# juanmc2005/diart

Hardware: NVIDIA H100
Metric: audio-seconds/sec (real-time factor) at 5s/0.5s step, batch 256 (higher is better)
Workload: dtype f32

## Files before the change

### diart_b200/_lib.py

```python
from __future__ import annotations

import ctypes as C
import os
from typing import Dict, Optional

import numpy as np
import torch

_HERE = os.path.dirname(os.path.abspath(__file__))
LIB_PATH = os.path.join(_HERE, "libdiartb200.so")

_lib: Optional[C.CDLL] = None


class DgTensor(C.Structure):
    _fields_ = [("name", C.c_char_p), ("data", C.c_void_p), ("numel", C.c_int64)]


_P = C.c_void_p
SIGNATURES = {
    "dg_last_error": (C.c_char_p, []),
    "dg_version": (C.c_int, []),
    "dg_launch_count": (C.c_int64, []),
    "dg_profile_enable": (C.c_int, [C.c_int]),
    "dg_profile_report": (C.c_int, [C.c_char_p, C.c_int]),
    "dg_selftest_gemm_tc": (C.c_int, [C.c_int, C.c_int, C.c_int, C.c_int, C.c_int, C.c_int, C.POINTER(C.c_float),
                                      C.POINTER(C.c_float)]),
    "dg_selftest_gemm_tc_grid": (C.c_int, [C.c_int, C.c_int, C.c_int, C.c_int, C.c_int, C.c_int, C.POINTER(C.c_int)]),
    "dg_selftest_gemm_tc_bounds": (C.c_int, [C.c_int, C.c_int, C.c_int, C.c_int, C.POINTER(C.c_int), C.POINTER(C.c_int),
                                             C.POINTER(C.c_int)]),
    "dg_selftest_wgmma_row_shift": (C.c_int, [C.c_int, C.POINTER(C.c_uint)]),
    "dg_selftest_gemm_tc_halo": (C.c_int, [C.c_int, C.c_int, C.c_int, C.c_int, C.c_int, C.c_int, C.POINTER(C.c_int),
                                           C.POINTER(C.c_int)]),
    "dg_selftest_split_f16_host": (C.c_int, [_P, C.c_longlong, _P, _P]),
    "dg_seg_create": (C.c_int, [C.POINTER(DgTensor), C.c_int, C.c_int, C.POINTER(_P)]),
    "dg_seg_dims": (C.c_int, [_P, C.c_int, C.POINTER(C.c_int), C.POINTER(C.c_int)]),
    "dg_seg_set_powerset": (C.c_int, [_P, C.c_int, C.c_int]),
    "dg_seg_forward": (C.c_int, [_P, _P, C.c_int, C.c_int, _P, _P]),
    "dg_seg_destroy": (C.c_int, [_P]),
    "dg_emb_create": (C.c_int, [C.POINTER(DgTensor), C.c_int, C.c_int, C.c_int, C.POINTER(_P)]),
    "dg_emb_dims": (C.c_int, [_P, C.c_int, C.POINTER(C.c_int), C.POINTER(C.c_int)]),
    "dg_emb_forward": (C.c_int, [_P, _P, _P, C.c_int, C.c_int, C.c_int, C.c_int, C.c_int, C.c_float, _P, _P]),
    "dg_emb_forward_rows": (C.c_int, [_P, _P, _P, C.c_int, C.c_int, C.c_int, _P, _P]),
    "dg_emb_destroy": (C.c_int, [_P]),
    "dg_emb_debug_trunk": (C.c_int, [_P, _P, C.c_int, C.c_int, C.c_int, _P, C.c_int64, _P]),
    "dg_seg_debug_stage": (C.c_int, [_P, _P, C.c_int, C.c_int, C.c_int, C.c_int, _P, C.c_int64, _P]),
    "dg_emb_debug_stage": (C.c_int, [_P, _P, _P, C.c_int, C.c_int, C.c_int, C.c_int, C.c_int, C.c_int, _P, C.c_int64, _P]),
    "dg_selftest_sinc_filters_host": (C.c_int, [_P, _P, _P]),
    "dg_selftest_fbank_tables_host": (C.c_int, [_P, _P]),
    "dg_osp": (C.c_int, [_P, C.c_int, C.c_int, C.c_int, C.c_float, C.c_float, C.c_int, _P, _P]),
    "dg_normalize_embeddings": (C.c_int, [_P, C.c_int, C.c_int, C.c_float, _P, _P]),
    "dg_cluster_create": (C.c_int, [C.c_int, C.c_int, C.c_double, C.c_double, C.c_double, C.c_int, C.POINTER(_P)]),
    "dg_cluster_set_metric": (C.c_int, [_P, C.c_int]),
    "dg_cluster_step": (C.c_int, [_P, _P, _P, C.c_int, C.c_int, C.c_int, _P, _P, _P]),
    "dg_cluster_reset": (C.c_int, [_P]),
# ... 149 lines not shown
```

### diart_b200/csrc/api.cu

```cuda
#include <math.h>
#include <stdlib.h>
#include <string.h>

#include <map>
#include <sstream>
#include <vector>

#include "host.cuh"

namespace dg {

static thread_local std::string g_err;
std::atomic<long long> g_launches{0};
thread_local int g_sm_limit = 0;
void set_error(const std::string& msg) { g_err = msg; }

struct ProfRec {
  std::string name;
  cudaEvent_t a, b;
};
static bool g_prof = false;
static std::vector<ProfRec> g_recs;
static const bool g_trace = getenv("DG_TRACE_LAUNCHES") && getenv("DG_TRACE_LAUNCHES")[0] == '1';
ProfScope::ProfScope(const char* name_, cudaStream_t st_) : on(g_prof), st(st_), a(nullptr), b(nullptr), name(name_) {
// ... 342 lines not shown
  ref.tap_boxes = 1;
  if (folded) {
    ref.Cin = Kf;
    ref.KW = 1;
    if ((rc = set_weights(ref, dWf))) return rc;
  }
  std::vector<unsigned char> first, cur;
  *equal = 1;
  for (int run = 0; run < 3; run++) {
    DG_CUDA(cudaMemset(dF.p, 0, f32_bytes + 4));
    DG_CUDA(cudaMemset(dOh.p, 0, plane_bytes + 4));
    DG_CUDA(cudaMemset(dOl.p, 0, plane_bytes + 4));
    DG_CUDA(cudaMemset(dPart.p, 0, part_bytes + 4));
    {
      SmLimit cap(run == 1 ? 3 : 0);
      if ((rc = launch_gemm_tc(run == 2 ? ref : t, nullptr))) return rc;
    }
    DG_CUDA(cudaDeviceSynchronize());
    cur.resize(f32_bytes + 2 * plane_bytes + part_bytes);
    DG_CUDA(cudaMemcpy(cur.data(), dF.p, f32_bytes, cudaMemcpyDeviceToHost));
    DG_CUDA(cudaMemcpy(cur.data() + f32_bytes, dOh.p, plane_bytes, cudaMemcpyDeviceToHost));
    DG_CUDA(cudaMemcpy(cur.data() + f32_bytes + plane_bytes, dOl.p, plane_bytes, cudaMemcpyDeviceToHost));
    DG_CUDA(cudaMemcpy(cur.data() + f32_bytes + 2 * plane_bytes, dPart.p, part_bytes, cudaMemcpyDeviceToHost));
    if (run == 0)
      first.swap(cur);
    else if (cur != first)
      *equal = 0;
  }
  return DG_OK;
}

extern "C" int dg_selftest_gemm_tc_bounds(int M, int Cin, int N, int epi, int* outside_unchanged, int* equal, int* refused) {
  const bool planes = epi == 1;
  if (M < 1 || Cin < 64 || Cin % 64 || N < 1 || N % (planes ? 32 : 4) || epi < 0 || epi > 2 || !outside_unchanged || !equal ||
      !refused) {
    set_error("dg_selftest_gemm_tc_bounds: bad arguments");
    return DG_EINVAL;
  }
  const int npad = N <= 64 && epi == 0 ? 64 : (N + 127) / 128 * 128, esize = planes ? 2 : 4;
  const int ldc = N + 40;
  const long long rows = (long long)M + 130;
  uint32_t seed = 4242u;
  auto rnd = [&]() {
    seed = seed * 1664525u + 1013904223u;
    return ((seed >> 8) & 0xFFFF) / 65536.f - 0.5f;
  };
// ... 64 lines not shown
```

### diart_b200/csrc/dg_common.cuh

```cuda
#pragma once
#include <cuda_runtime.h>
#include <stdint.h>
#include <stdio.h>

#include <atomic>
#include <string>
#include <vector>

namespace dg {

void set_error(const std::string& msg);
extern std::atomic<long long> g_launches;
extern thread_local int g_sm_limit;
inline int usable_sms() {
  int dev = 0, sms = 132;
  cudaGetDevice(&dev);
  cudaDeviceGetAttribute(&sms, cudaDevAttrMultiProcessorCount, dev);
  return (g_sm_limit > 0 && g_sm_limit < sms) ? g_sm_limit : sms;
}

#define DG_CUDA(expr)                                                                   \
  do {                                                                                  \
    cudaError_t _e = (expr);                                                            \
    if (_e != cudaSuccess) {                                                            \
// ... 100 lines not shown
  float* out_f32;
  void* out_hi;
  void* out_lo;
  int ldc;
  int epi;
  const char* tag;
  const int* tap_off;
  int Wp, Hp, Wop, Hop, stride2, relu;
  const void* res_hi;
  const void* res_lo;
  const float* pool_w;
  float* pool_part;
  int pool_item_rows, pool_K;
  int pool3_T, pool3_tile_rows;
  int tap_boxes;
};
inline int gemm_tc_pool3_tile_rows(int item_rows) {
  for (int t = 126; t >= 96; t -= 3)
    if (item_rows % t == 0) return t;
  return 0;
}
int launch_gemm_tc(const TcGemm& g, cudaStream_t st);
bool gemm_tc_halo(const TcGemm& g);
int selftest_wgmma_row_shift(int base_offset_mode, unsigned* ok_shifts);
int launch_split_ex(const float* x, long long rows_out, int C, int ld_in, int ld_out, int pool, int item_rows,
                    const float* sc, const float* sh, void* hi, void* lo, cudaStream_t st, const int* skip_flag = nullptr);
void split_weights_host(const float* w, int N, int Npad, int K, uint16_t* hi, uint16_t* lo, float scale = 1.f);
float weight_plane_scale(const float* w, size_t n);
uint16_t host_f32_to_h16(float f);
float host_h16_to_f32(uint16_t h);
int sinc_tc_rows_per_item(const Geom& g);
size_t sinc_tc_plane_elems(int B, const Geom& g);
void sinc_tc_pack_filters(const float* filt, uint16_t* planes );
void sinc_tc_affine_consts(const float* filt, float beta, float* cf);
int launch_sinc_prep(const float* wav, const float* mean, const float* rstd, int B, const Geom& g, void* planes_hi,
                     void* planes_lo, cudaStream_t st, const int* skip_flag = nullptr);
int launch_sinc0_tc(float gamma, const float* cf_dev, const void* w_planes, int B, const Geom& g, const void* planes_hi,
                    const void* planes_lo, float* p0, cudaStream_t st, const int* skip_flag = nullptr);
struct SincStreamGeom {
  int Ls;
  int P;
  int rows;
  size_t plane;
};
SincStreamGeom sinc_stream_geom(int B, const Geom& g, int hop);
int launch_overlap_check(const float* wav, int B, int S, int hop, int* flag, cudaStream_t st);
// ... 148 lines not shown
```

### diart_b200/csrc/gemm_tc.cu

```cuda
#include <cuda.h>
#include <cuda_bf16.h>
#include <math.h>
#include <stdlib.h>
#include <string.h>

#include <algorithm>
#include <map>
#include <mutex>
#include <string>
#include <utility>
#include <vector>

#include "dg_common.cuh"
#include "tc_ptx.cuh"

namespace dg {

constexpr int TC_BM = 128, TC_BK = 32, TC_THREADS = 384;
constexpr int TC_SMEM_MAX = 227 * 1024;

struct TcArgs {
  long long M;
  int N;
  int m_tiles, n_tiles;
  int KW, dil, cin_blocks;
  const float* bias;
  const float* bn_scale;
  const float* bn_shift;
  float* out_f32;
  __nv_bfloat16* out_hi;
  __nv_bfloat16* out_lo;
  int ldc;
  float acc_scale;
  int tap_off[9];
  int Wp, Hp, Wop, Hop, stride2, relu;
  const __nv_bfloat16* res_hi;
  const __nv_bfloat16* res_lo;
  const float* pool_w;
  float* pool_part;
  int pool_item_rows, pool_K;
  int tile_rows, pool3_T;
  unsigned* tile_ctr;
  int halo_rows;
  int cin;
  int wblocks;
  int halo_bytes;
  int op_bytes;
};

enum TcEpi { TC_BIAS_F32 = 0, TC_LEAKY_BN_SPLIT = 1, TC_LEAKY_BN_F32 = 2, TC_CONV2D = 3, TC_POOL = 4, TC_MAXPOOL3 = 5 };

__host__ __device__ constexpr bool tc_pooling(int epi) { return epi == TC_POOL || epi == TC_MAXPOOL3; }
__host__ __device__ constexpr bool tc_box_store(int epi) { return epi == TC_BIAS_F32 || epi == TC_LEAKY_BN_SPLIT || epi == TC_LEAKY_BN_F32; }

template <int BN>
struct TcSmem {
  static constexpr int A_BYTES = TC_BM * TC_BK * 2;
  static constexpr int W_BYTES = BN * TC_BK * 2;
  static constexpr int STAGE_BYTES = 2 * A_BYTES + 2 * W_BYTES;
  static constexpr int W_STAGE_BYTES = 2 * W_BYTES;
  static constexpr int NSTAGE = BN == 128 ? 4 : 6;
  static constexpr int NSTAGE_HALO = BN == 128 ? 5 : 6;
  __host__ static int halo_bytes(int cin, int rows) { return (2 * ((cin + 31) / 32) * rows * 64 + 1023) / 1024 * 1024; }
  __host__ static int halo_op_bytes(int cin, int rows) { return 2 * halo_bytes(cin, rows) + NSTAGE_HALO * W_STAGE_BYTES; }
  static constexpr int BAR_BYTES = 256;
  static constexpr int PARAM_FLOATS = 3 * BN;
  static constexpr int CHUNK_W = 64;
  static constexpr int CHUNK_FLOATS = CHUNK_W / 32 * TC_BM * 33;
  __host__ __device__ static constexpr int extra_floats(int epi) { return epi == TC_POOL ? 128 * 4 + 4 * 2 * 8 * 32 : (epi == TC_MAXPOOL3 ? 4 * 2 * 2 * 32 : 0); }
  __host__ __device__ static constexpr int consumer_floats(int epi) { return PARAM_FLOATS + (tc_pooling(epi) ? CHUNK_FLOATS + extra_floats(epi) : 0); }
  static constexpr int ACC_LD = BN + 4;
  static constexpr int BOX_BYTES = TC_BM * 128;
  __host__ __device__ static constexpr int stage_tile_bytes(int epi) {
    return tc_pooling(epi) ? 0 : (epi == TC_CONV2D ? TC_BM * ACC_LD * 4 : TC_BM * BN * 4);
  }
  __host__ __device__ static constexpr int total(int epi, int op_bytes = NSTAGE * STAGE_BYTES) {
    return op_bytes + stage_tile_bytes(epi) + BAR_BYTES + 2 * consumer_floats(epi) * 4 + 1024;
  }
};
static_assert(TcSmem<128>::total(TC_POOL) <= TC_SMEM_MAX && TcSmem<64>::total(TC_MAXPOOL3) <= TC_SMEM_MAX &&
              TcSmem<128>::total(TC_CONV2D) <= TC_SMEM_MAX && TcSmem<64>::total(TC_CONV2D) <= TC_SMEM_MAX &&
              TcSmem<32>::total(TC_CONV2D) <= TC_SMEM_MAX && TcSmem<128>::total(TC_BIAS_F32) <= TC_SMEM_MAX,
              "gemm_tc: shared memory");

template <int BN, int EPI>
__device__ __forceinline__ void tc_stage_params(const TcArgs& a, float* params, int bar, int n0, int et) {
  named_sync(bar, 128);
  for (int i = et; i < BN; i += 128) {
    const int n = n0 + i;
    const bool ok = n < a.N;
    params[i] = (ok && a.bias) ? a.bias[n] : 0.f;
    constexpr bool has_bn = EPI != TC_BIAS_F32;
    params[BN + i] = (ok && has_bn) ? a.bn_scale[n] * (EPI == TC_CONV2D ? a.acc_scale : 1.f) : 1.f;
    params[2 * BN + i] = (ok && has_bn) ? a.bn_shift[n] : 0.f;
  }
  named_sync(bar, 128);
}

template <int BN, int EPI>
__device__ __forceinline__ void tc_box_epilogue(const TcArgs& a, const float* params, float (&acc)[2][BN / 2],
                                                uint32_t tile, int quad, int lane) {
  using S = TcSmem<BN>;
  const int r0 = 16 * quad + (lane >> 2), sw = lane >> 2, cq = lane & 3;
#pragma unroll
  for (int j = 0; j < BN / 8; j++) {
    const int col = 8 * j + 2 * cq;
    const float2 bias = *reinterpret_cast<const float2*>(params + col);
    float2 bsc = make_float2(1.f, 1.f), bsh = make_float2(0.f, 0.f);
    if (EPI != TC_BIAS_F32) {
      bsc = *reinterpret_cast<const float2*>(params + BN + col);
      bsh = *reinterpret_cast<const float2*>(params + 2 * BN + col);
    }
#pragma unroll
    for (int h = 0; h < 2; h++) {
#pragma unroll
      for (int e2 = 0; e2 < 2; e2++) {
        const int row = 64 * h + r0 + 8 * e2;
        float x0 = fmaf(acc[h][4 * j + 2 * e2], a.acc_scale, bias.x);
        float x1 = fmaf(acc[h][4 * j + 2 * e2 + 1], a.acc_scale, bias.y);
        if (EPI != TC_BIAS_F32) {
          x0 = fmaf(leaky(x0), bsc.x, bsh.x);
          x1 = fmaf(leaky(x1), bsc.y, bsh.y);
        }
        if (EPI == TC_LEAKY_BN_SPLIT) {
          uint16_t h0, l0, h1, l1;
          split_h16(x0, h0, l0);
          split_h16(x1, h1, l1);
          const int off = (j / 8) * S::BOX_BYTES + row * 128 + (((j & 7) ^ sw) << 4) + 4 * cq;
          st_shared_u32(tile + off, pack_u16x2(h0, h1));
          st_shared_u32(tile + (BN / 64) * S::BOX_BYTES + off, pack_u16x2(l0, l1));
        } else {
          const int q = 2 * (j & 3) + (cq >> 1);
          const int off = (j / 4) * S::BOX_BYTES + row * 128 + ((q ^ sw) << 4) + 8 * (cq & 1);
          st_shared_v2(tile + off, x0, x1);
        }
      }
    }
  }
}

__device__ __forceinline__ void acc_ld32(const float* p, uint32_t (&r)[32]) {
#pragma unroll
  for (int i = 0; i < 8; i++) {
    const float4 v = reinterpret_cast<const float4*>(p)[i];
    r[4 * i] = __float_as_uint(v.x);
    r[4 * i + 1] = __float_as_uint(v.y);
    r[4 * i + 2] = __float_as_uint(v.z);
    r[4 * i + 3] = __float_as_uint(v.w);
  }
}

template <int BN>
__device__ __forceinline__ void tc_conv2d_epilogue_tile(const TcArgs& a, const float* params, const float* acc_row,
                                                        long long mt, int n0, int quad, int lane) {
    const long long m = mt * TC_BM + quad * 32 + lane;
    long long mo = m;
// ... 204 lines not shown
                }
              }
            }
#pragma unroll
            for (int sg = 0; sg < 2; sg++) {
              stg[((rg * 2 + sg) * 2 + 0) * 32 + col] = s1[sg];
              stg[((rg * 2 + sg) * 2 + 1) * 32 + col] = s2[sg];
            }
          }
          named_sync(bar, 128);
          {
            const int col = et & 31, q = et >> 5, sg = q >> 1, j = q & 1, n = n0 + c + col;
            const float tot = ((stg[((0 * 2 + sg) * 2 + j) * 32 + col] + stg[((1 * 2 + sg) * 2 + j) * 32 + col]) +
                               stg[((2 * 2 + sg) * 2 + j) * 32 + col]) + stg[((3 * 2 + sg) * 2 + j) * 32 + col];
            if (n < a.N) a.pool_part[(((size_t)mt * 2 + sg) * 2 + j) * a.N + n] = tot;
          }
          named_sync(bar, 128);
          continue;
        }
      }
    }
}

template <int BN, int EPI, bool HALO>
__global__ void __launch_bounds__(TC_THREADS, 1)
gemm_tc_kernel(const __grid_constant__ CUtensorMap tmA_hi, const __grid_constant__ CUtensorMap tmA_lo,
               const __grid_constant__ CUtensorMap tmW_hi, const __grid_constant__ CUtensorMap tmW_lo,
               const __grid_constant__ CUtensorMap tmC0, const __grid_constant__ CUtensorMap tmC1, TcArgs a) {
  using S = TcSmem<BN>;
  constexpr bool POOLING = tc_pooling(EPI);
  constexpr int NSTAGE = HALO ? S::NSTAGE_HALO : S::NSTAGE;
  extern __shared__ unsigned char smem_raw[];
  unsigned char* smem = reinterpret_cast<unsigned char*>((reinterpret_cast<uintptr_t>(smem_raw) + 1023) & ~uintptr_t(1023));
  unsigned char* ring = HALO ? smem + 2 * a.halo_bytes : smem;
  constexpr int RING_STAGE = HALO ? S::W_STAGE_BYTES : S::STAGE_BYTES;
  unsigned char* tile_s = smem + a.op_bytes;
  uint64_t* bars = reinterpret_cast<uint64_t*>(tile_s + S::stage_tile_bytes(EPI));
  uint64_t* full = bars;
  uint64_t* empty = bars + NSTAGE;
  uint64_t* tile_full = bars + 2 * NSTAGE;
  uint64_t* tile_empty = tile_full + 2;
  uint64_t* halo_full = tile_empty + 2;
  uint64_t* halo_empty = halo_full + 2;
  volatile int* tile_idx = reinterpret_cast<volatile int*>(halo_empty + 2);
  float* cons = reinterpret_cast<float*>(reinterpret_cast<unsigned char*>(bars) + S::BAR_BYTES);

  const int warp = __shfl_sync(0xffffffffu, (int)(threadIdx.x >> 5), 0), lane = threadIdx.x & 31;
  const int wg = warp >> 2;
  const int num_tiles = a.m_tiles * a.n_tiles;
  const int kblocks = HALO ? a.wblocks : a.KW * a.cin_blocks;
  const int halo_box = a.halo_rows * 64, halo_cb = (a.cin + 31) / 32;

  if (threadIdx.x == 0) {
    for (int s = 0; s < NSTAGE; s++) {
      mbar_init(&full[s], 1);
      mbar_init(&empty[s], 1);
    }
    for (int c = 0; c < 2; c++) {
      mbar_init(&tile_full[c], 1);
      mbar_init(&tile_empty[c], 128);
      mbar_init(&halo_full[c], 1);
      mbar_init(&halo_empty[c], 1);
    }
    asm volatile("fence.mbarrier_init.release.cluster;" ::: "memory");
  }
  __syncthreads();

  if (wg == 0) {
    setmaxnreg_dec<HALO ? 48 : 40>();
    if (threadIdx.x == 0) {
      int stage = 0, phase = 0, next = 0;
      bool halo_next = false;
      for (int i = 0, tile = blockIdx.x;; i++) {
        const int c = i & 1;
        mbar_wait(&tile_empty[c], ((i >> 1) & 1) ^ 1);
        if (tile >= num_tiles) {
          tile_idx[c] = -1;
          mbar_arrive(&tile_full[c]);
          mbar_wait(&tile_empty[c ^ 1], (((i + 1) >> 1) & 1) ^ 1);
          tile_idx[c ^ 1] = -2;
          mbar_arrive(&tile_full[c ^ 1]);
          break;
        }
        tile_idx[c] = tile;
        mbar_arrive(&tile_full[c]);
        const int mt = tile / a.n_tiles, nt = tile - mt * a.n_tiles;
        const int m0 = mt * (EPI == TC_MAXPOOL3 ? a.tile_rows : TC_BM), n0 = nt * BN;
        if constexpr (HALO) {
          auto load_halo = [&](int cc, int r0) {
            unsigned char* hs = smem + cc * a.halo_bytes;
            mbar_expect_tx(&halo_full[cc], 2 * halo_cb * halo_box);
            for (int cb = 0; cb < halo_cb; cb++) {
              tma_load_2d(hs + cb * halo_box, &tmA_hi, cb * TC_BK, r0, &halo_full[cc]);
              tma_load_2d(hs + (halo_cb + cb) * halo_box, &tmA_lo, cb * TC_BK, r0, &halo_full[cc]);
            }
// ... 9 lines not shown
          for (int kb = 0; kb < kblocks; kb++) {
            const long long t0 = clock64();
            for (;;) {
              if (!halo_next && next < num_tiles && mbar_test_wait(&halo_empty[c ^ 1], next_par)) {
                load_halo(c ^ 1, next_m0);
                halo_next = true;
              }
              if (mbar_test_wait(&empty[stage], phase ^ 1)) break;
              if (clock64() - t0 > 4000000000LL) __trap();
            }
            unsigned char* st = ring + stage * RING_STAGE;
            mbar_expect_tx(&full[stage], S::W_STAGE_BYTES);
            tma_load_2d(st, &tmW_hi, kb * TC_BK, n0, &full[stage]);
            tma_load_2d(st + S::W_BYTES, &tmW_lo, kb * TC_BK, n0, &full[stage]);
            if (++stage == NSTAGE) {
              stage = 0;
              phase ^= 1;
            }
          }
        }
        for (int j = 0; j < (HALO ? 0 : a.KW); j++) {
          for (int cb = 0; cb < a.cin_blocks; cb++) {
            mbar_wait(&empty[stage], phase ^ 1);
            unsigned char* st = smem + stage * S::STAGE_BYTES;
            mbar_expect_tx(&full[stage], S::STAGE_BYTES);
            const int kcol = (j * a.cin_blocks + cb) * TC_BK;
            tma_load_2d(st, &tmA_hi, cb * TC_BK, m0 + a.tap_off[j], &full[stage]);
            tma_load_2d(st + S::A_BYTES, &tmA_lo, cb * TC_BK, m0 + a.tap_off[j], &full[stage]);
            tma_load_2d(st + 2 * S::A_BYTES, &tmW_hi, kcol, n0, &full[stage]);
            tma_load_2d(st + 2 * S::A_BYTES + S::W_BYTES, &tmW_lo, kcol, n0, &full[stage]);
            if (++stage == NSTAGE) {
              stage = 0;
              phase ^= 1;
            }
          }
        }
        if (!HALO) next = POOLING ? (int)gridDim.x + (int)atomicAdd(&a.tile_ctr[0], 1u) : tile + (int)gridDim.x;
        tile = next;
      }
      if (POOLING) {
        __threadfence();
        if (atomicAdd(&a.tile_ctr[1], 1u) == gridDim.x - 1) {
          atomicExch(&a.tile_ctr[0], 0u);
          atomicExch(&a.tile_ctr[1], 0u);
        }
      }
    }
    return;
  }
  setmaxnreg_inc<HALO ? 224 : 232>();
  const int c = wg - 1, quad = warp & 3, et = threadIdx.x - 128 * wg;
  float* params = cons + c * S::consumer_floats(EPI);
  float* chunk = params + S::PARAM_FLOATS;
  float* pool_stage = chunk + S::CHUNK_FLOATS;
  const int bar = 1 + c, turn = 3 + c, turn_other = 3 + (c ^ 1), acc_free = 5 + c, acc_free_other = 5 + (c ^ 1);
  if (c == 1) {
    named_arrive(3, 256);
    if (!POOLING) named_arrive(5, 256);
  }
  for (int n = 0;; n++) {
    mbar_wait(&tile_full[c], n & 1);
    const int tile = tile_idx[c];
    mbar_arrive(&tile_empty[c]);
    if (tc_box_store(EPI) && tile >= 0 && (a.n_tiles > 1 || n == 0))
      tc_stage_params<BN, EPI>(a, params, bar, (tile - tile / a.n_tiles * a.n_tiles) * BN, et);
    named_sync(turn, 256);
    if (tile < 0) {
      if (tile == -1) {
        named_arrive(turn_other, 256);
        if (!POOLING) named_sync(acc_free, 256);
      }
      break;
    }
    const int pos = (2 * n + c) * kblocks;
    int stage = pos % NSTAGE, phase = (pos / NSTAGE) & 1;
    float acc[2][BN / 2];
#pragma unroll
    for (int i = 0; i < BN / 2; i++) acc[0][i] = acc[1][i] = 0.f;
    uint32_t htap = 0;
    int hch = 0;
    if constexpr (HALO) mbar_wait(&halo_full[c], n & 1);
    const uint32_t hs = smem_u32(smem + c * a.halo_bytes);
    for (int kb = 0; kb < kblocks; kb++) {
      mbar_wait(&full[stage], phase);
      const uint32_t sa = smem_u32(ring + stage * RING_STAGE);
      const uint32_t sw = HALO ? sa : sa + 2 * S::A_BYTES;
      const uint64_t w_hi = wg_desc_sw64(sw), w_lo = wg_desc_sw64(sw + S::W_BYTES);
      constexpr uint64_t HALF = (uint64_t)((64 * TC_BK * 2) >> 4);
      wg_fence_acc(acc[0]);
      wg_fence_acc(acc[1]);
      wg_fence();
#pragma unroll
      for (int ks = 0; ks < TC_BK / 16; ks++) {
        const uint64_t adv = (uint64_t)((ks * 32) >> 4);
        uint64_t a_hi, a_lo;
        if constexpr (HALO) {
          const uint32_t aa = hs + (uint32_t)(hch >> 5) * halo_box + (uint32_t)(hch & 31) * 2 + htap;
          a_hi = wg_desc_sw64(aa);
          a_lo = wg_desc_sw64(aa + halo_cb * halo_box);
          hch += 16;
          const bool next_tap = hch == a.cin;
          hch = next_tap ? 0 : hch;
          htap += next_tap ? a.dil * 64 : 0;
        } else {
          a_hi = wg_desc_sw64(sa) + adv;
          a_lo = wg_desc_sw64(sa + S::A_BYTES) + adv;
        }
#pragma unroll
        for (int h = 0; h < 2; h++) {
          wgmma_ss<BN>(acc[h], a_lo + h * HALF, w_hi + adv, (kb | ks) != 0);
          wgmma_ss<BN>(acc[h], a_hi + h * HALF, w_lo + adv, 1);
          wgmma_ss<BN>(acc[h], a_hi + h * HALF, w_hi + adv, 1);
        }
      }
      wg_commit();
      wg_wait<1>();
      wg_fence_acc(acc[0]);
      wg_fence_acc(acc[1]);
      if (kb > 0 && et == 0) mbar_arrive(&empty[stage == 0 ? NSTAGE - 1 : stage - 1]);
      if (++stage == NSTAGE) {
        stage = 0;
        phase ^= 1;
      }
    }
    named_arrive(turn_other, 256);
    wg_wait<0>();
    wg_fence_acc(acc[0]);
    wg_fence_acc(acc[1]);
    if (et == 0) mbar_arrive(&empty[stage == 0 ? NSTAGE - 1 : stage - 1]);
    if (HALO && et == 0) mbar_arrive(&halo_empty[c]);
    const int mt = tile / a.n_tiles, nt = tile - mt * a.n_tiles;
    const bool stage_params = a.n_tiles > 1 || n == 0;
    if constexpr (POOLING) {
      tc_pool_epilogue_tile<BN, EPI>(a, params, chunk, pool_stage, acc, bar, mt, nt * BN, quad, lane, et, stage_params);
    } else if constexpr (EPI == TC_CONV2D) {
      float* acc_s = reinterpret_cast<float*>(tile_s);
      named_sync(acc_free, 256);
#pragma unroll
      for (int h = 0; h < 2; h++) {
        const int r0 = 64 * h + 16 * quad + (lane >> 2);
#pragma unroll
        for (int j = 0; j < BN / 8; j++) {
          const int col = 8 * j + 2 * (lane & 3);
          *reinterpret_cast<float2*>(acc_s + r0 * S::ACC_LD + col) = make_float2(acc[h][4 * j], acc[h][4 * j + 1]);
          *reinterpret_cast<float2*>(acc_s + (r0 + 8) * S::ACC_LD + col) = make_float2(acc[h][4 * j + 2], acc[h][4 * j + 3]);
        }
      }
      named_sync(bar, 128);
      if (stage_params) tc_stage_params<BN, EPI>(a, params, bar, nt * BN, et);
      tc_conv2d_epilogue_tile<BN>(a, params, acc_s + et * S::ACC_LD, mt, nt * BN, quad, lane);
      named_arrive(acc_free_other, 256);
    } else {
      named_sync(acc_free, 256);
      tc_box_epilogue<BN, EPI>(a, params, acc, smem_u32(tile_s), quad, lane);
      fence_proxy_async_smem();
      named_sync(bar, 128);
      if (et == 0) {
        const int m0 = mt * TC_BM, n0 = nt * BN;
        if (EPI == TC_LEAKY_BN_SPLIT) {
#pragma unroll
          for (int b = 0; b < BN / 64; b++) {
            if (n0 + 64 * b >= a.N) break;
            tma_store_2d(&tmC0, tile_s + b * S::BOX_BYTES, n0 + 64 * b, m0);
            tma_store_2d(&tmC1, tile_s + (BN / 64 + b) * S::BOX_BYTES, n0 + 64 * b, m0);
          }
        } else {
#pragma unroll
          for (int b = 0; b < BN / 32; b++) {
            if (n0 + 32 * b >= a.N) break;
            tma_store_2d(&tmC0, tile_s + b * S::BOX_BYTES, n0 + 32 * b, m0);
          }
        }
        bulk_commit();
// ... 57 lines not shown
  }
  void* base = nullptr;
  if (cudaGetSymbolAddress(&base, g_tc_tile_ctr) != cudaSuccess) {
    set_error("gemm_tc: cannot address the tile counters");
    return nullptr;
  }
  return static_cast<unsigned*>(base) + 2 * slot;
}

static int tc_bn(const TcGemm& g) { return g.epi == TC_MAXPOOL3 || (g.Npad == 64 && g.epi == TC_BIAS_F32) ? 64 : 128; }
static int tc_halo_rows(const TcGemm& g) {
  return (TC_BM + (g.KW - ((g.KW * g.Cin) % 32 ? 0 : 1)) * g.dil + 7) / 8 * 8;
}
template <int BN>
static int tc_halo_smem(const TcGemm& g) { return TcSmem<BN>::total(g.epi, TcSmem<BN>::halo_op_bytes(g.Cin, tc_halo_rows(g))); }

bool gemm_tc_halo(const TcGemm& g) {
  if (g.tap_boxes || g.epi == TC_CONV2D || g.tap_off || g.KW < 2 || g.dil < 1 || g.Cin % 16 || g.Cin > 128 ||
      tc_halo_rows(g) > 256)
    return false;
  return (tc_bn(g) == 64 ? tc_halo_smem<64>(g) : tc_halo_smem<128>(g)) <= TC_SMEM_MAX;
}

static int tc_setup(const TcGemm& g, int bn, int epi, bool halo, CUtensorMap* maps, TcArgs& a) {
  const int Ktot = g.KW * g.Cin, bk = TC_BK, a_rows = halo ? tc_halo_rows(g) : TC_BM;
  if (make_map(&maps[0], g.A_hi, g.Mtot, g.Cin, g.lda, bk, a_rows) || make_map(&maps[1], g.A_lo, g.Mtot, g.Cin, g.lda, bk, a_rows) ||
      make_map(&maps[2], g.W_hi, g.Npad, Ktot, Ktot, bk, bn) || make_map(&maps[3], g.W_lo, g.Npad, Ktot, Ktot, bk, bn))
    return -2;
  memset(&maps[4], 0, 2 * sizeof(CUtensorMap));
  if (epi == TC_LEAKY_BN_SPLIT) {
    if (make_map(&maps[4], g.out_hi, g.M, g.N, g.ldc, 64, TC_BM) || make_map(&maps[5], g.out_lo, g.M, g.N, g.ldc, 64, TC_BM))
      return -2;
  } else if (tc_box_store(epi)) {
    if (make_map(&maps[4], g.out_f32, g.M, g.N, g.ldc, 32, TC_BM, true)) return -2;
  }
  a = TcArgs{};
  a.M = g.M; a.N = g.N; a.n_tiles = (g.N + bn - 1) / bn;
  a.tile_rows = epi == TC_MAXPOOL3 ? g.pool3_tile_rows : TC_BM;
  a.pool3_T = g.pool3_T;
  a.m_tiles = (int)((g.M + a.tile_rows - 1) / a.tile_rows);
  a.KW = g.KW; a.dil = g.dil; a.cin_blocks = g.Cin / bk;
  a.bias = g.bias; a.bn_scale = g.bn_scale; a.bn_shift = g.bn_shift;
  a.out_f32 = g.out_f32; a.out_hi = reinterpret_cast<__nv_bfloat16*>(g.out_hi);
  a.out_lo = reinterpret_cast<__nv_bfloat16*>(g.out_lo); a.ldc = g.ldc;
  a.acc_scale = g.w_scale > 0.f ? 1.f / g.w_scale : 1.f;
  for (int j = 0; j < 9; j++) a.tap_off[j] = j < g.KW ? (g.tap_off ? g.tap_off[j] : j * g.dil) : 0;
  a.Wp = g.Wp; a.Hp = g.Hp; a.Wop = g.Wop; a.Hop = g.Hop; a.stride2 = g.stride2; a.relu = g.relu;
  a.res_hi = reinterpret_cast<const __nv_bfloat16*>(g.res_hi);
  a.res_lo = reinterpret_cast<const __nv_bfloat16*>(g.res_lo);
  a.pool_w = g.pool_w; a.pool_part = g.pool_part; a.pool_item_rows = g.pool_item_rows; a.pool_K = g.pool_K;
  a.cin = g.Cin;
  if (halo) {
    a.halo_rows = a_rows;
    a.wblocks = (Ktot + bk - 1) / bk;
    a.halo_bytes = bn == 64 ? TcSmem<64>::halo_bytes(g.Cin, a_rows) : TcSmem<128>::halo_bytes(g.Cin, a_rows);
    a.op_bytes = bn == 64 ? TcSmem<64>::halo_op_bytes(g.Cin, a_rows) : TcSmem<128>::halo_op_bytes(g.Cin, a_rows);
  } else {
    a.op_bytes = bn == 128 ? TcSmem<128>::NSTAGE * TcSmem<128>::STAGE_BYTES
                           : (bn == 64 ? TcSmem<64>::NSTAGE * TcSmem<64>::STAGE_BYTES : TcSmem<32>::NSTAGE * TcSmem<32>::STAGE_BYTES);
  }
  return 0;
}

static int tc_grid(const TcArgs& a) {
  const int sms = usable_sms();
  const int tiles = a.m_tiles * a.n_tiles;
  return tiles < sms ? tiles : sms;
}

template <int BN, int EPI, bool HALO>
static int launch_tc(const TcGemm& g, cudaStream_t st) {
  using S = TcSmem<BN>;
  CUtensorMap m[6];
  TcArgs a;
  if (tc_setup(g, BN, EPI, HALO, m, a)) return -2;
  if (tc_pooling(EPI) && !(a.tile_ctr = tile_counter(st))) return -2;
  auto kern = gemm_tc_kernel<BN, EPI, HALO>;
  static bool attr_done[64] = {};
  if (first_use_on_device(attr_done))
    DG_CUDA(cudaFuncSetAttribute(kern, cudaFuncAttributeMaxDynamicSharedMemorySize, HALO ? TC_SMEM_MAX : S::total(EPI)));
  kern<<<tc_grid(a), TC_THREADS, S::total(EPI, a.op_bytes), st>>>(m[0], m[1], m[2], m[3], m[4], m[5], a);
  DG_LAUNCHED();
  return 0;
}

template <int BN, int EPI>
static int launch_tc(const TcGemm& g, cudaStream_t st) {
  return gemm_tc_halo(g) ? launch_tc<BN, EPI, true>(g, st) : launch_tc<BN, EPI, false>(g, st);
}

int launch_gemm_tc(const TcGemm& g, cudaStream_t st) {
  ProfScope _ps(g.tag ? g.tag : "gemm_tc", st);
  if (g.Cin % (gemm_tc_halo(g) ? 16 : 64) || g.lda % 8 || g.ldc % (g.epi == TC_LEAKY_BN_SPLIT ? 8 : 4) ||
      (g.Npad % 128 && g.Npad != 64 && g.Npad != 32) || g.KW < 1 || g.KW > 9) {
    set_error("gemm_tc: Cin must be a multiple of 64 (a Conv1d of 2..9 taps over at most 128 channels whose tile halo fits "
              "in shared memory, e.g. Cin 80: a multiple of 16), A pitch a multiple of 8, output pitch a multiple of 4 "
              "(8 for 16-bit planes), padded N 32, 64 or a multiple of 128, at most 9 taps");
    return -1;
  }
  if (g.epi == TC_LEAKY_BN_SPLIT && g.N % 32) {
    set_error("gemm_tc (planes): N must be a multiple of 32");
    return -1;
  }
  if (tc_box_store(g.epi)) {
    const bool planes = g.epi == TC_LEAKY_BN_SPLIT;
    const uintptr_t base = planes ? ((uintptr_t)g.out_hi | (uintptr_t)g.out_lo) : (uintptr_t)g.out_f32;
    if (!base || (planes && (!g.out_hi || !g.out_lo)) || base % 16 || g.ldc < g.N || g.M >= (1LL << 31)) {
      set_error("gemm_tc: the output needs a 16-byte aligned base, a pitch of at least N and fewer than 2^31 rows");
      return -1;
    }
  }
  if (g.epi == TC_CONV2D) {
    if (g.ldc % 32 || g.N % 32 || g.Wp < 3 || g.Hp < 3 || (!g.out_hi && !g.out_f32) || g.M >= (1LL << 31)) {
      set_error("gemm_tc (conv2d): channel counts must be multiples of 32");
      return -1;
    }
    if (g.Npad == 32) return launch_tc<32, TC_CONV2D, false>(g, st);
    if (g.Npad == 64) return launch_tc<64, TC_CONV2D, false>(g, st);
    return launch_tc<128, TC_CONV2D, false>(g, st);
  }
// ... 220 lines not shown
```

### include/diart_b200.h

```cpp
#ifndef DIART_B200_H
#define DIART_B200_H

#include <stddef.h>
#include <stdint.h>

#ifdef __cplusplus
extern "C" {
#endif

#define DG_OK 0
#define DG_EINVAL (-1)
#define DG_ECUDA (-2)
#define DG_EWEIGHT (-3)
#define DG_ENCCL (-4)

typedef struct dg_tensor {
  const char* name;
  const float* data;
  int64_t numel;
} dg_tensor;

typedef struct dg_seg dg_seg;
typedef struct dg_emb dg_emb;
typedef struct dg_cluster dg_cluster;
// ... 156 lines not shown
int dg_selftest_multi_frames_host(int slots, int max_wps, int out_chunk, int out_step, int n_rates, const int32_t* rates,
                                  int n_ops, const int32_t* ops, int32_t* result, int64_t* records, int cap, int* n_records);
int dg_selftest_multi_staging_host(int slots, int C, int n_ops, const int32_t* ops, const float* samples_host, int32_t* result,
                                   float* rings_host);
int dg_multi_create_vad(dg_seg* seg, int chunk_samples, int step_samples, int max_streams, int max_windows_per_stream,
                        double tau, int num_windows, const double* hamming_host, dg_multi** out);

typedef struct dg_resample dg_resample;
int dg_resample_create(int orig_rate, int new_rate, const float* taps_host, int width, int device, dg_resample** out);
int64_t dg_resample_out_len(const dg_resample* h, int64_t num_samples);
int dg_resample_forward(dg_resample* h, const float* in_dev, int B, int64_t L, float* out_dev, void* stream);
int dg_resample_destroy(dg_resample* h);
int dg_stream_create_resampled(int chunk_samples, int step_samples, dg_resample* rs, int max_windows, int device,
                               dg_stream** out);
int dg_stream_crop_host(dg_stream* h, int n, const int64_t* ranges_host, float* out_host);

int64_t dg_launch_count(void);
int dg_profile_enable(int enable);
int dg_selftest_gemm_tc(int M, int Cin, int KW, int dil, int N, int epi, float* max_abs_diff, float* out_rms);
int dg_selftest_gemm_tc_grid(int M, int Cin, int KW, int dil, int N, int epi, int* equal);
int dg_selftest_gemm_tc_bounds(int M, int Cin, int N, int epi, int* outside_unchanged, int* equal, int* refused);
int dg_selftest_wgmma_row_shift(int base_offset_mode, unsigned* ok_shifts);
int dg_selftest_gemm_tc_halo(int M, int Cin, int KW, int dil, int N, int epi, int* equal, int* halo);
int dg_selftest_split_f16_host(const float* x, long long n, unsigned short* hi, unsigned short* lo);
int dg_selftest_sinc_filters_host(const float* low_hz, const float* band_hz, float* filters);
int dg_selftest_fbank_tables_host(float* frame_operator, float* mel_banks);
int dg_profile_report(char* buf, int cap);

int dg_cluster_record_len(const dg_cluster* h);
int dg_cluster_export_delta(dg_cluster* h, double* record_dev, void* stream);
int dg_cluster_merge(dg_cluster* h, const double* records_dev , int world, int rank,
                     int32_t* maps_dev , int n_maps, void* stream);
int dg_pipeline_identity_export(dg_pipeline* h, double* record_dev, void* stream);
int dg_pipeline_identity_merge(dg_pipeline* h, const double* records_dev, int world, int rank, void* stream);

#ifdef __cplusplus
}
#endif
#endif
```

Before: 23120.

## Add weight-resident mode to tensor-core GEMM keeping the full weight slice in shared memory

Adds a weight-resident variant of the persistent wgmma GEMM for 1-tap, BN=128, box-store epilogues. Each CTA loads its entire N-column weight slice into shared memory once and then streams only A tiles through a smaller ring. The grid is pinned so each CTA keeps a fixed n-tile. The epilogue is split into narrower column passes to shrink the staging tile. This cuts repeated weight TMA traffic per k-block but leaves fewer pipeline stages, can reduce grid size, and serializes epilogue stores.

```diff
diff --git a/diart_b200/_lib.py b/diart_b200/_lib.py
--- a/diart_b200/_lib.py
+++ b/diart_b200/_lib.py
@@ -31,6 +31,8 @@
                                              C.POINTER(C.c_int)]),
     "dg_selftest_wgmma_row_shift": (C.c_int, [C.c_int, C.POINTER(C.c_uint)]),
     "dg_selftest_gemm_tc_halo": (C.c_int, [C.c_int, C.c_int, C.c_int, C.c_int, C.c_int, C.c_int, C.POINTER(C.c_int),
+                                           C.POINTER(C.c_int)]),
+    "dg_selftest_gemm_tc_wres": (C.c_int, [C.c_int, C.c_int, C.c_int, C.c_int, C.c_int, C.POINTER(C.c_int),
                                            C.POINTER(C.c_int)]),
     "dg_selftest_split_f16_host": (C.c_int, [_P, C.c_longlong, _P, _P]),
     "dg_seg_create": (C.c_int, [C.POINTER(DgTensor), C.c_int, C.c_int, C.POINTER(_P)]),
diff --git a/diart_b200/csrc/api.cu b/diart_b200/csrc/api.cu
--- a/diart_b200/csrc/api.cu
+++ b/diart_b200/csrc/api.cu
@@ -388,6 +388,71 @@
     DG_CUDA(cudaMemcpy(cur.data() + f32_bytes, dOh.p, plane_bytes, cudaMemcpyDeviceToHost));
     DG_CUDA(cudaMemcpy(cur.data() + f32_bytes + plane_bytes, dOl.p, plane_bytes, cudaMemcpyDeviceToHost));
     DG_CUDA(cudaMemcpy(cur.data() + f32_bytes + 2 * plane_bytes, dPart.p, part_bytes, cudaMemcpyDeviceToHost));
+    if (run == 0)
+      first.swap(cur);
+    else if (cur != first)
+      *equal = 0;
+  }
+  return DG_OK;
+}
+
+extern "C" int dg_selftest_gemm_tc_wres(int M, int Cin, int N, int epi, int sm_cap, int* equal, int* wres) {
+  if (M < 1 || Cin < 64 || Cin % 64 || N < 1 || N % 32 || epi < 0 || epi > 2 || sm_cap < 0 || !equal || !wres) {
+    set_error("dg_selftest_gemm_tc_wres: bad arguments");
+    return DG_EINVAL;
+  }
+  const int npad = (N + 127) / 128 * 128;
+  uint32_t seed = 5151u;
+  auto rnd = [&]() {
+    seed = seed * 1664525u + 1013904223u;
+    return ((seed >> 8) & 0xFFFF) / 65536.f - 0.5f;
+  };
+  std::vector<float> A((size_t)M * Cin), Wnk((size_t)N * Cin), bias(N), bsc(N), bsh(N);
+  for (auto& v : A) v = 2.f * rnd();
+  for (auto& v : Wnk) v = 0.25f * rnd();
+  for (int n = 0; n < N; n++) {
+    bias[n] = rnd();
+    bsc[n] = 1.f + rnd();
+    bsh[n] = rnd();
+  }
+  const size_t f32_bytes = epi == 1 ? 0 : (size_t)M * N * 4, plane_bytes = epi == 1 ? (size_t)M * N * 2 : 0;
+  DevBuf dA, dAh, dAl, dB, dS, dH, dF, dOh, dOl;
+  WeightPlanes dW;
+  if (upload(dA, A) || upload(dB, bias) || upload(dS, bsc) || upload(dH, bsh) || upload_split(dW, Wnk, N, npad, Cin) ||
+      dAh.ensure((size_t)M * Cin * 2) || dAl.ensure((size_t)M * Cin * 2) || dF.ensure(f32_bytes + 4) ||
+      dOh.ensure(plane_bytes + 4) || dOl.ensure(plane_bytes + 4))
+    return DG_ECUDA;
+  int rc;
+  if ((rc = launch_split_ex(dA.as<float>(), M, Cin, Cin, Cin, 0, 1, nullptr, nullptr, dAh.p, dAl.p, nullptr))) return rc;
+  TcGemm t{};
+  t.A_hi = dAh.p; t.A_lo = dAl.p; t.lda = Cin; t.Cin = Cin; t.KW = 1; t.dil = 1; t.Mtot = M; t.M = M;
+  t.N = N; t.bias = dB.as<float>(); t.bn_scale = dS.as<float>(); t.bn_shift = dH.as<float>(); t.ldc = N;
+  t.epi = epi; t.tag = "selftest_tc_wres";
+  t.out_f32 = f32_bytes ? dF.as<float>() : nullptr;
+  t.out_hi = plane_bytes ? dOh.p : nullptr;
+  t.out_lo = plane_bytes ? dOl.p : nullptr;
+  if ((rc = set_weights(t, dW))) return rc;
+  {
+    SmLimit cap(sm_cap);
+    *wres = gemm_tc_wres(t) ? 1 : 0;
+  }
+  TcGemm ref = t;
+  ref.tap_boxes = 1;
+  std::vector<unsigned char> first, cur;
+  *equal = 1;
+  for (int run = 0; run < 2; run++) {
+    DG_CUDA(cudaMemset(dF.p, 0, f32_bytes + 4));
+    DG_CUDA(cudaMemset(dOh.p, 0, plane_bytes + 4));
+    DG_CUDA(cudaMemset(dOl.p, 0, plane_bytes + 4));
+    {
+      SmLimit cap(run == 0 ? sm_cap : 0);
+      if ((rc = launch_gemm_tc(run == 0 ? t : ref, nullptr))) return rc;
+    }
+    DG_CUDA(cudaDeviceSynchronize());
+    cur.resize(f32_bytes + 2 * plane_bytes);
+    DG_CUDA(cudaMemcpy(cur.data(), dF.p, f32_bytes, cudaMemcpyDeviceToHost));
+    DG_CUDA(cudaMemcpy(cur.data() + f32_bytes, dOh.p, plane_bytes, cudaMemcpyDeviceToHost));
+    DG_CUDA(cudaMemcpy(cur.data() + f32_bytes + plane_bytes, dOl.p, plane_bytes, cudaMemcpyDeviceToHost));
     if (run == 0)
       first.swap(cur);
     else if (cur != first)
diff --git a/diart_b200/csrc/dg_common.cuh b/diart_b200/csrc/dg_common.cuh
--- a/diart_b200/csrc/dg_common.cuh
+++ b/diart_b200/csrc/dg_common.cuh
@@ -146,6 +146,7 @@
 }
 int launch_gemm_tc(const TcGemm& g, cudaStream_t st);
 bool gemm_tc_halo(const TcGemm& g);
+bool gemm_tc_wres(const TcGemm& g);
 int selftest_wgmma_row_shift(int base_offset_mode, unsigned* ok_shifts);
 int launch_split_ex(const float* x, long long rows_out, int C, int ld_in, int ld_out, int pool, int item_rows,
                     const float* sc, const float* sh, void* hi, void* lo, cudaStream_t st, const int* skip_flag = nullptr);
diff --git a/diart_b200/csrc/gemm_tc.cu b/diart_b200/csrc/gemm_tc.cu
--- a/diart_b200/csrc/gemm_tc.cu
+++ b/diart_b200/csrc/gemm_tc.cu
@@ -46,6 +46,7 @@
   int wblocks;
   int halo_bytes;
   int op_bytes;
+  int nstage;
 };
 
 enum TcEpi { TC_BIAS_F32 = 0, TC_LEAKY_BN_SPLIT = 1, TC_LEAKY_BN_F32 = 2, TC_CONV2D = 3, TC_POOL = 4, TC_MAXPOOL3 = 5 };
@@ -61,6 +62,11 @@
   static constexpr int W_STAGE_BYTES = 2 * W_BYTES;
   static constexpr int NSTAGE = BN == 128 ? 4 : 6;
   static constexpr int NSTAGE_HALO = BN == 128 ? 5 : 6;
+  static constexpr int A_STAGE_BYTES = 2 * A_BYTES;
+  static constexpr int NSTAGE_WRES = 6;
+  __host__ __device__ static constexpr int wres_cols(int epi) { return epi == TC_LEAKY_BN_SPLIT ? 64 : 32; }
+  __host__ __device__ static constexpr int wres_tile_bytes(int epi) { return epi == TC_LEAKY_BN_SPLIT ? 2 * BOX_BYTES : BOX_BYTES; }
+  __host__ static int wres_slice_bytes(int cin_blocks) { return cin_blocks * W_STAGE_BYTES; }
   __host__ static int halo_bytes(int cin, int rows) { return (2 * ((cin + 31) / 32) * rows * 64 + 1023) / 1024 * 1024; }
   __host__ static int halo_op_bytes(int cin, int rows) { return 2 * halo_bytes(cin, rows) + NSTAGE_HALO * W_STAGE_BYTES; }
   static constexpr int BAR_BYTES = 256;
@@ -77,6 +83,9 @@
   __host__ __device__ static constexpr int total(int epi, int op_bytes = NSTAGE * STAGE_BYTES) {
     return op_bytes + stage_tile_bytes(epi) + BAR_BYTES + 2 * consumer_floats(epi) * 4 + 1024;
   }
+  __host__ static int total_wres(int epi, int op_bytes) {
+    return op_bytes + wres_tile_bytes(epi) + BAR_BYTES + 2 * consumer_floats(epi) * 4 + 1024;
+  }
 };
 static_assert(TcSmem<128>::total(TC_POOL) <= TC_SMEM_MAX && TcSmem<64>::total(TC_MAXPOOL3) <= TC_SMEM_MAX &&
               TcSmem<128>::total(TC_CONV2D) <= TC_SMEM_MAX && TcSmem<64>::total(TC_CONV2D) <= TC_SMEM_MAX &&
@@ -97,13 +106,13 @@
   named_sync(bar, 128);
 }
 
-template <int BN, int EPI>
+template <int BN, int EPI, int C0 = 0, int CW = BN>
 __device__ __forceinline__ void tc_box_epilogue(const TcArgs& a, const float* params, float (&acc)[2][BN / 2],
                                                 uint32_t tile, int quad, int lane) {
   using S = TcSmem<BN>;
   const int r0 = 16 * quad + (lane >> 2), sw = lane >> 2, cq = lane & 3;
 #pragma unroll
-  for (int j = 0; j < BN / 8; j++) {
+  for (int j = C0 / 8; j < (C0 + CW) / 8; j++) {
     const int col = 8 * j + 2 * cq;
     const float2 bias = *reinterpret_cast<const float2*>(params + col);
     float2 bsc = make_float2(1.f, 1.f), bsh = make_float2(0.f, 0.f);
@@ -126,12 +135,12 @@
           uint16_t h0, l0, h1, l1;
           split_h16(x0, h0, l0);
           split_h16(x1, h1, l1);
-          const int off = (j / 8) * S::BOX_BYTES + row * 128 + (((j & 7) ^ sw) << 4) + 4 * cq;
+          const int off = ((j - C0 / 8) / 8) * S::BOX_BYTES + row * 128 + (((j & 7) ^ sw) << 4) + 4 * cq;
           st_shared_u32(tile + off, pack_u16x2(h0, h1));
-          st_shared_u32(tile + (BN / 64) * S::BOX_BYTES + off, pack_u16x2(l0, l1));
+          st_shared_u32(tile + (CW / 64) * S::BOX_BYTES + off, pack_u16x2(l0, l1));
         } else {
           const int q = 2 * (j & 3) + (cq >> 1);
-          const int off = (j / 4) * S::BOX_BYTES + row * 128 + ((q ^ sw) << 4) + 8 * (cq & 1);
+          const int off = ((j - C0 / 8) / 4) * S::BOX_BYTES + row * 128 + ((q ^ sw) << 4) + 8 * (cq & 1);
           st_shared_v2(tile + off, x0, x1);
         }
       }
@@ -382,26 +391,29 @@
     }
 }
 
-template <int BN, int EPI, bool HALO>
+template <int BN, int EPI, bool HALO, bool WRES = false>
 __global__ void __launch_bounds__(TC_THREADS, 1)
 gemm_tc_kernel(const __grid_constant__ CUtensorMap tmA_hi, const __grid_constant__ CUtensorMap tmA_lo,
                const __grid_constant__ CUtensorMap tmW_hi, const __grid_constant__ CUtensorMap tmW_lo,
                const __grid_constant__ CUtensorMap tmC0, const __grid_constant__ CUtensorMap tmC1, TcArgs a) {
   using S = TcSmem<BN>;
   constexpr bool POOLING = tc_pooling(EPI);
-  constexpr int NSTAGE = HALO ? S::NSTAGE_HALO : S::NSTAGE;
+  static_assert(!WRES || (BN == 128 && tc_box_store(EPI) && !HALO), "gemm_tc: weight-resident mode");
+  constexpr int NSTAGE = HALO ? S::NSTAGE_HALO : (WRES ? S::NSTAGE_WRES : S::NSTAGE);
+  const int nstage = WRES ? a.nstage : NSTAGE;
   extern __shared__ unsigned char smem_raw[];
   unsigned char* smem = reinterpret_cast<unsigned char*>((reinterpret_cast<uintptr_t>(smem_raw) + 1023) & ~uintptr_t(1023));
-  unsigned char* ring = HALO ? smem + 2 * a.halo_bytes : smem;
-  constexpr int RING_STAGE = HALO ? S::W_STAGE_BYTES : S::STAGE_BYTES;
+  unsigned char* ring = HALO ? smem + 2 * a.halo_bytes : (WRES ? smem + S::W_STAGE_BYTES * a.cin_blocks : smem);
+  constexpr int RING_STAGE = HALO ? S::W_STAGE_BYTES : (WRES ? S::A_STAGE_BYTES : S::STAGE_BYTES);
   unsigned char* tile_s = smem + a.op_bytes;
-  uint64_t* bars = reinterpret_cast<uint64_t*>(tile_s + S::stage_tile_bytes(EPI));
+  uint64_t* bars = reinterpret_cast<uint64_t*>(tile_s + (WRES ? S::wres_tile_bytes(EPI) : S::stage_tile_bytes(EPI)));
   uint64_t* full = bars;
   uint64_t* empty = bars + NSTAGE;
   uint64_t* tile_full = bars + 2 * NSTAGE;
   uint64_t* tile_empty = tile_full + 2;
   uint64_t* halo_full = tile_empty + 2;
   uint64_t* halo_empty = halo_full + 2;
+  uint64_t* w_full = halo_full;
   volatile int* tile_idx = reinterpret_cast<volatile int*>(halo_empty + 2);
   float* cons = reinterpret_cast<float*>(reinterpret_cast<unsigned char*>(bars) + S::BAR_BYTES);
 
@@ -431,6 +443,14 @@
     if (threadIdx.x == 0) {
       int stage = 0, phase = 0, next = 0;
       bool halo_next = false;
+      if constexpr (WRES) {
+        const int n0 = (int)(blockIdx.x % (unsigned)a.n_tiles) * BN;
+        mbar_expect_tx(w_full, a.cin_blocks * S::W_STAGE_BYTES);
+        for (int kb = 0; kb < a.cin_blocks; kb++) {
+          tma_load_2d(smem + kb * S::W_STAGE_BYTES, &tmW_hi, kb * TC_BK, n0, w_full);
+          tma_load_2d(smem + kb * S::W_STAGE_BYTES + S::W_BYTES, &tmW_lo, kb * TC_BK, n0, w_full);
+        }
+      }
       for (int i = 0, tile = blockIdx.x;; i++) {
         const int c = i & 1;
         mbar_wait(&tile_empty[c], ((i >> 1) & 1) ^ 1);
@@ -486,14 +506,16 @@
         for (int j = 0; j < (HALO ? 0 : a.KW); j++) {
           for (int cb = 0; cb < a.cin_blocks; cb++) {
             mbar_wait(&empty[stage], phase ^ 1);
-            unsigned char* st = smem + stage * S::STAGE_BYTES;
-            mbar_expect_tx(&full[stage], S::STAGE_BYTES);
+            unsigned char* st = WRES ? ring + stage * RING_STAGE : smem + stage * S::STAGE_BYTES;
+            mbar_expect_tx(&full[stage], RING_STAGE);
             const int kcol = (j * a.cin_blocks + cb) * TC_BK;
             tma_load_2d(st, &tmA_hi, cb * TC_BK, m0 + a.tap_off[j], &full[stage]);
             tma_load_2d(st + S::A_BYTES, &tmA_lo, cb * TC_BK, m0 + a.tap_off[j], &full[stage]);
-            tma_load_2d(st + 2 * S::A_BYTES, &tmW_hi, kcol, n0, &full[stage]);
-            tma_load_2d(st + 2 * S::A_BYTES + S::W_BYTES, &tmW_lo, kcol, n0, &full[stage]);
-            if (++stage == NSTAGE) {
+            if (!WRES) {
+              tma_load_2d(st + 2 * S::A_BYTES, &tmW_hi, kcol, n0, &full[stage]);
+              tma_load_2d(st + 2 * S::A_BYTES + S::W_BYTES, &tmW_lo, kcol, n0, &full[stage]);
+            }
+            if (++stage == nstage) {
               stage = 0;
               phase ^= 1;
             }
@@ -526,7 +548,7 @@
     mbar_wait(&tile_full[c], n & 1);
     const int tile = tile_idx[c];
     mbar_arrive(&tile_empty[c]);
-    if (tc_box_store(EPI) && tile >= 0 && (a.n_tiles > 1 || n == 0))
+    if (tc_box_store(EPI) && tile >= 0 && ((!WRES && a.n_tiles > 1) || n == 0))
       tc_stage_params<BN, EPI>(a, params, bar, (tile - tile / a.n_tiles * a.n_tiles) * BN, et);
     named_sync(turn, 256);
     if (tile < 0) {
@@ -537,18 +559,21 @@
       break;
     }
     const int pos = (2 * n + c) * kblocks;
-    int stage = pos % NSTAGE, phase = (pos / NSTAGE) & 1;
+    int stage = pos % nstage, phase = (pos / nstage) & 1;
     float acc[2][BN / 2];
 #pragma unroll
     for (int i = 0; i < BN / 2; i++) acc[0][i] = acc[1][i] = 0.f;
     uint32_t htap = 0;
     int hch = 0;
     if constexpr (HALO) mbar_wait(&halo_full[c], n & 1);
+    if constexpr (WRES) {
+      if (n == 0) mbar_wait(w_full, 0);
+    }
     const uint32_t hs = smem_u32(smem + c * a.halo_bytes);
     for (int kb = 0; kb < kblocks; kb++) {
       mbar_wait(&full[stage], phase);
       const uint32_t sa = smem_u32(ring + stage * RING_STAGE);
-      const uint32_t sw = HALO ? sa : sa + 2 * S::A_BYTES;
+      const uint32_t sw = HALO ? sa : (WRES ? smem_u32(smem) + kb * S::W_STAGE_BYTES : sa + 2 * S::A_BYTES);
       const uint64_t w_hi = wg_desc_sw64(sw), w_lo = wg_desc_sw64(sw + S::W_BYTES);
       constexpr uint64_t HALF = (uint64_t)((64 * TC_BK * 2) >> 4);
       wg_fence_acc(acc[0]);
@@ -581,8 +606,8 @@
       wg_wait<1>();
       wg_fence_acc(acc[0]);
       wg_fence_acc(acc[1]);
-      if (kb > 0 && et == 0) mbar_arrive(&empty[stage == 0 ? NSTAGE - 1 : stage - 1]);
-      if (++stage == NSTAGE) {
+      if (kb > 0 && et == 0) mbar_arrive(&empty[stage == 0 ? nstage - 1 : stage - 1]);
+      if (++stage == nstage) {
         stage = 0;
         phase ^= 1;
       }
@@ -591,7 +616,7 @@
     wg_wait<0>();
     wg_fence_acc(acc[0]);
     wg_fence_acc(acc[1]);
-    if (et == 0) mbar_arrive(&empty[stage == 0 ? NSTAGE - 1 : stage - 1]);
+    if (et == 0) mbar_arrive(&empty[stage == 0 ? nstage - 1 : stage - 1]);
     if (HALO && et == 0) mbar_arrive(&halo_empty[c]);
     const int mt = tile / a.n_tiles, nt = tile - mt * a.n_tiles;
     const bool stage_params = a.n_tiles > 1 || n == 0;
@@ -613,6 +638,31 @@
       named_sync(bar, 128);
       if (stage_params) tc_stage_params<BN, EPI>(a, params, bar, nt * BN, et);
       tc_conv2d_epilogue_tile<BN>(a, params, acc_s + et * S::ACC_LD, mt, nt * BN, quad, lane);
+      named_arrive(acc_free_other, 256);
+    } else if constexpr (WRES) {
+      constexpr int CW = S::wres_cols(EPI);
+      static_assert(BN / CW <= 4, "gemm_tc: weight-resident epilogue passes");
+      named_sync(acc_free, 256);
+#pragma unroll
+      for (int p = 0; p < BN / CW; p++) {
+        if (p) named_sync(bar, 128);
+        if (p == 0) tc_box_epilogue<BN, EPI, 0, CW>(a, params, acc, smem_u32(tile_s), quad, lane);
+        if (p == 1) tc_box_epilogue<BN, EPI, CW, CW>(a, params, acc, smem_u32(tile_s), quad, lane);
+        if (p == 2) tc_box_epilogue<BN, EPI, 2 * CW, CW>(a, params, acc, smem_u32(tile_s), quad, lane);
+        if (p == 3) tc_box_epilogue<BN, EPI, 3 * CW, CW>(a, params, acc, smem_u32(tile_s), quad, lane);
+        fence_proxy_async_smem();
+        named_sync(bar, 128);
+        if (et == 0) {
+          const int m0 = mt * TC_BM, n0 = nt * BN + CW * p;
+          if (n0 < a.N) {
+            tma_store_2d(&tmC0, tile_s, n0, m0);
+            if (EPI == TC_LEAKY_BN_SPLIT) tma_store_2d(&tmC1, tile_s + S::BOX_BYTES, n0, m0);
+          }
+          bulk_commit();
+          bulk_wait_read_all();
+        }
+      }
+      __syncwarp();
       named_arrive(acc_free_other, 256);
     } else {
       named_sync(acc_free, 256);
@@ -716,7 +766,21 @@
   return (tc_bn(g) == 64 ? tc_halo_smem<64>(g) : tc_halo_smem<128>(g)) <= TC_SMEM_MAX;
 }
 
-static int tc_setup(const TcGemm& g, int bn, int epi, bool halo, CUtensorMap* maps, TcArgs& a) {
+static int tc_wres_nstage(int epi, int cin) {
+  using S = TcSmem<128>;
+  const int op = S::wres_slice_bytes(cin / TC_BK);
+  const int n = (TC_SMEM_MAX - S::total_wres(epi, op)) / S::A_STAGE_BYTES;
+  return n < S::NSTAGE_WRES ? n : S::NSTAGE_WRES;
+}
+
+bool gemm_tc_wres(const TcGemm& g) {
+  if (g.tap_boxes || g.tap_off || g.KW != 1 || !tc_box_store(g.epi) || tc_bn(g) != 128 || g.Cin % 64 ||
+      tc_wres_nstage(g.epi, g.Cin) < 2)
+    return false;
+  return usable_sms() >= (g.N + 127) / 128;
+}
+
+static int tc_setup(const TcGemm& g, int bn, int epi, bool halo, CUtensorMap* maps, TcArgs& a, bool wres = false) {
   const int Ktot = g.KW * g.Cin, bk = TC_BK, a_rows = halo ? tc_halo_rows(g) : TC_BM;
   if (make_map(&maps[0], g.A_hi, g.Mtot, g.Cin, g.lda, bk, a_rows) || make_map(&maps[1], g.A_lo, g.Mtot, g.Cin, g.lda, bk, a_rows) ||
       make_map(&maps[2], g.W_hi, g.Npad, Ktot, Ktot, bk, bn) || make_map(&maps[3], g.W_lo, g.Npad, Ktot, Ktot, bk, bn))
@@ -749,6 +813,9 @@
     a.wblocks = (Ktot + bk - 1) / bk;
     a.halo_bytes = bn == 64 ? TcSmem<64>::halo_bytes(g.Cin, a_rows) : TcSmem<128>::halo_bytes(g.Cin, a_rows);
     a.op_bytes = bn == 64 ? TcSmem<64>::halo_op_bytes(g.Cin, a_rows) : TcSmem<128>::halo_op_bytes(g.Cin, a_rows);
+  } else if (wres) {
+    a.nstage = tc_wres_nstage(epi, g.Cin);
+    a.op_bytes = TcSmem<128>::wres_slice_bytes(a.cin_blocks) + a.nstage * TcSmem<128>::A_STAGE_BYTES;
   } else {
     a.op_bytes = bn == 128 ? TcSmem<128>::NSTAGE * TcSmem<128>::STAGE_BYTES
                            : (bn == 64 ? TcSmem<64>::NSTAGE * TcSmem<64>::STAGE_BYTES : TcSmem<32>::NSTAGE * TcSmem<32>::STAGE_BYTES);
@@ -756,30 +823,38 @@
   return 0;
 }
 
-static int tc_grid(const TcArgs& a) {
+static int tc_grid(const TcArgs& a, bool wres = false) {
   const int sms = usable_sms();
   const int tiles = a.m_tiles * a.n_tiles;
+  if (wres) {
+    const int per = sms / a.n_tiles;
+    return a.n_tiles * (a.m_tiles < per ? a.m_tiles : per);
+  }
   return tiles < sms ? tiles : sms;
 }
 
-template <int BN, int EPI, bool HALO>
+template <int BN, int EPI, bool HALO, bool WRES = false>
 static int launch_tc(const TcGemm& g, cudaStream_t st) {
   using S = TcSmem<BN>;
   CUtensorMap m[6];
   TcArgs a;
-  if (tc_setup(g, BN, EPI, HALO, m, a)) return -2;
+  if (tc_setup(g, BN, EPI, HALO, m, a, WRES)) return -2;
   if (tc_pooling(EPI) && !(a.tile_ctr = tile_counter(st))) return -2;
-  auto kern = gemm_tc_kernel<BN, EPI, HALO>;
+  auto kern = gemm_tc_kernel<BN, EPI, HALO, WRES>;
   static bool attr_done[64] = {};
   if (first_use_on_device(attr_done))
-    DG_CUDA(cudaFuncSetAttribute(kern, cudaFuncAttributeMaxDynamicSharedMemorySize, HALO ? TC_SMEM_MAX : S::total(EPI)));
-  kern<<<tc_grid(a), TC_THREADS, S::total(EPI, a.op_bytes), st>>>(m[0], m[1], m[2], m[3], m[4], m[5], a);
+    DG_CUDA(cudaFuncSetAttribute(kern, cudaFuncAttributeMaxDynamicSharedMemorySize, HALO || WRES ? TC_SMEM_MAX : S::total(EPI)));
+  const int smem = WRES ? S::total_wres(EPI, a.op_bytes) : S::total(EPI, a.op_bytes);
+  kern<<<tc_grid(a, WRES), TC_THREADS, smem, st>>>(m[0], m[1], m[2], m[3], m[4], m[5], a);
   DG_LAUNCHED();
   return 0;
 }
 
 template <int BN, int EPI>
 static int launch_tc(const TcGemm& g, cudaStream_t st) {
+  if constexpr (BN == 128 && tc_box_store(EPI)) {
+    if (gemm_tc_wres(g)) return launch_tc<BN, EPI, false, true>(g, st);
+  }
   return gemm_tc_halo(g) ? launch_tc<BN, EPI, true>(g, st) : launch_tc<BN, EPI, false>(g, st);
 }
 
@@ -790,6 +865,10 @@
     set_error("gemm_tc: Cin must be a multiple of 64 (a Conv1d of 2..9 taps over at most 128 channels whose tile halo fits "
               "in shared memory, e.g. Cin 80: a multiple of 16), A pitch a multiple of 8, output pitch a multiple of 4 "
               "(8 for 16-bit planes), padded N 32, 64 or a multiple of 128, at most 9 taps");
+    return -1;
+  }
+  if (((uintptr_t)g.A_hi | (uintptr_t)g.A_lo | (uintptr_t)g.W_hi | (uintptr_t)g.W_lo) % 16) {
+    set_error("gemm_tc: the operand planes need 16-byte aligned bases");
     return -1;
   }
   if (g.epi == TC_LEAKY_BN_SPLIT && g.N % 32) {
diff --git a/include/diart_b200.h b/include/diart_b200.h
--- a/include/diart_b200.h
+++ b/include/diart_b200.h
@@ -202,6 +202,7 @@
 int dg_selftest_gemm_tc_bounds(int M, int Cin, int N, int epi, int* outside_unchanged, int* equal, int* refused);
 int dg_selftest_wgmma_row_shift(int base_offset_mode, unsigned* ok_shifts);
 int dg_selftest_gemm_tc_halo(int M, int Cin, int KW, int dil, int N, int epi, int* equal, int* halo);
+int dg_selftest_gemm_tc_wres(int M, int Cin, int N, int epi, int sm_cap, int* equal, int* wres);
 int dg_selftest_split_f16_host(const float* x, long long n, unsigned short* hi, unsigned short* lo);
 int dg_selftest_sinc_filters_host(const float* low_hz, const float* band_hz, float* filters);
 int dg_selftest_fbank_tables_host(float* frame_operator, float* mel_banks);
```

Measured after the change: 23350 (median of 6 runs). About the same (+1.0%).
